# shresthasagar/quantized_spectrum_cartography

Measured on AMD Instinct MI355X. Metric: MLE grad-steps/sec + SLF NMSE, 512x512x256 R=8, higher is better.
Workload: dtype f32

## Files before the change

quantized_spectrum_cartography_amd/csrc/qsc_pass.cuh:

```cuda
#pragma once
#include <algorithm>

#include "qsc_common.cuh"

using namespace qsc;

namespace {

#if QSC_DEBUG
__device__ int g_qsc_dbg_line = 0;
inline int dbg_line_read(bool clear) {
  int line = 0;
  if (hipMemcpyFromSymbol(&line, HIP_SYMBOL(g_qsc_dbg_line), sizeof(int)) != hipSuccess) return -2;
  if (clear && line) {
    const int zero = 0;
    if (hipMemcpyToSymbol(HIP_SYMBOL(g_qsc_dbg_line), &zero, sizeof(int)) != hipSuccess) return -2;
  }
  return line;
}
#endif

constexpr int kSBlock = 256;
constexpr int kSWaves = kSBlock / 64;
#ifndef QSC_CPASS_BLOCK
#define QSC_CPASS_BLOCK 512
#endif
constexpr int kCBlock = QSC_CPASS_BLOCK;
constexpr int kCParts = kCBlock / 64;
#ifndef QSC_CPART_MIN_CHUNKS
#define QSC_CPART_MIN_CHUNKS 1.5
#endif
constexpr int kFBlock = 1024;

#ifndef QSC_SPASS_WAVES
#define QSC_SPASS_WAVES 4
#endif
#ifndef QSC_EARLY_WAVES
#define QSC_EARLY_WAVES 16
#endif
__device__ __forceinline__ void prio_level(int lvl) {
  if (lvl >= 3)
    __builtin_amdgcn_s_setprio(3);
  else if (lvl == 2)
    __builtin_amdgcn_s_setprio(2);
  else if (lvl == 1)
    __builtin_amdgcn_s_setprio(1);
  else
    __builtin_amdgcn_s_setprio(0);
}
#ifndef QSC_FUSED_WAVES
#define QSC_FUSED_WAVES 16
#endif
#ifndef QSC_CPASS_WAVES
#define QSC_CPASS_WAVES 4
#endif
struct PartRange {
  int j0, j1, js;
};
__device__ inline PartRange part_range(int W4, int p, int np) {
  return PartRange{(W4 * p) / np, (W4 * (p + 1)) / np, 1};
}
#ifndef QSC_CPASS_TILE
#define QSC_CPASS_TILE 1
#endif
#ifndef QSC_CTILE_MAXW
#define QSC_CTILE_MAXW 16
#endif
#ifndef QSC_CTILE_W16
#define QSC_CTILE_W16 8
#endif
#ifndef QSC_CTILE_SREG
#define QSC_CTILE_SREG 4
#endif
#ifndef QSC_CTILE_CT
#define QSC_CTILE_CT 1
#endif
template <int RP, int W>
struct Occ {
  static constexpr int v = (RP > 8) ? (W > 4 ? 4 : W) : W;
};
#ifndef QSC_SPASS_BPC8
#define QSC_SPASS_BPC8 3
#endif
template <int RP, int EB, int W>
struct OccS {
  static constexpr int v = (RP > 8) ? (W > 2 ? 2 : W) : (RP == 8) ? QSC_SPASS_BPC8 : W;
};

template <int RP>
struct Pitch {
  static constexpr int v = (RP == 4) ? 4 : RP + 4;
};
template <int RP, int KIND>
// ... 327 lines not shown
#pragma unroll
    for (int j = 0; j < RP / 2; ++j) acc[j] = fma2(splat2(gb), ob[j], acc[j]);
  }
}

template <int RP, typename E, int KIND, bool LOG>
__device__ __forceinline__ void half_chunk(const typename Ent<E>::V2& v, const f2v (&own)[RP / 2],
                                           const float* __restrict__ tab,
                                           const float2* __restrict__ edges, const Lik& lk,
                                           f2v (&acc)[RP / 2], f2v& nll) {
  uint32_t e[2];
  Ent<E>::unpack2(v, e);
  f2v oa[RP / 2], ob[RP / 2];
  f2v tha, thb, pq;
  pair_rows<RP, E, KIND, 0>(e[0], e[1], own, tab, oa, ob, tha, thb, lk);
  pair_math<RP, E, KIND, LOG>(e[0], e[1], own, oa, ob, tha, thb, edges, lk, acc, nll, pq);
}

constexpr int kGroup = 4;
constexpr int kSchedQ = 16;

template <typename V4>
__device__ __forceinline__ void load_group(const V4* __restrict__ src, uint32_t lo, int row, int jb,
                                           int js, int jlast, V4 (&b)[kGroup]) {
#pragma unroll
  for (int i = 0; i < kGroup; ++i) {
    const int j = min(jb + i * js, jlast);
    b[i] = ld_lane(src + (int64_t)j * row, lo);
  }
}

template <int RP, typename E, int KIND, bool LOG>
__device__ __forceinline__ void walk_groups(const typename Ent<E>::V4* __restrict__ src,
                                            uint32_t lo, int row, int jb, int j1, int js,
                                            typename Ent<E>::V4 (&b)[kGroup],
                                            const f2v (&own)[RP / 2],
                                            const float* __restrict__ tab,
                                            const float2* __restrict__ edges, const Lik& lk,
                                            f2v (&acc)[RP / 2], f2v& nll) {
  using V4 = typename Ent<E>::V4;
  const int jlast = max(j1 - 1, 0);
  const int jfirst = jb, jspan = max(j1 - jb, 1);
  auto fair = [&]() { prio_level(3 - min(3, (4 * (jb - jfirst)) / jspan)); };
  const uint32_t off = sr_addr<E, KIND>() ? lds_off(tab) : 0u;
  f2v ra[RP / 2], rb[RP / 2];
  f2v tra, trb;
  {
    uint32_t e[4];
    ent_rows4<RP, E, KIND>(b[0], off, e);
    pair_rows<RP, E, KIND, 1>(e[0], e[1], own, tab, ra, rb, tra, trb, lk);
  }
  for (;;) {
    fair();
    const int jn = jb + kGroup * js;
    const bool more = jn < j1;
    V4 nb[kGroup];
    load_group(src, lo, row, jn, js, jlast, nb);
#pragma unroll
    for (int i = 0; i < kGroup; ++i)
      if (jb + i * js < j1) {
        uint32_t e[4];
        ent_rows4<RP, E, KIND>(b[i], off, e);
        f2v xa[RP / 2], xb[RP / 2];
        f2v txa, txb, pqa, pqb;
        pair_rows<RP, E, KIND, 1>(e[2], e[3], own, tab, xa, xb, txa, txb, lk);
        pair_math<RP, E, KIND, LOG>(e[0], e[1], own, ra, rb, tra, trb, edges, lk, acc, nll, pqa);
        if (i + 1 < kGroup) {
          uint32_t f[4];
          ent_rows4<RP, E, KIND>(b[i + 1], off, f);
          pair_rows<RP, E, KIND, 1>(f[0], f[1], own, tab, ra, rb, tra, trb, lk);
        }
        pair_math<RP, E, KIND, LOG>(e[2], e[3], own, xa, xb, txa, txb, edges, lk, acc, nll, pqb);
        if constexpr (is_sr(KIND)) {
          const f2v pp = pqa * pqb;
          nll.x -= __builtin_amdgcn_logf(pp.x * pp.y);
        }
      }
    if (!more) break;
#pragma unroll
    for (int i = 0; i < kGroup; ++i) b[i] = nb[i];
    {
      uint32_t e[4];
      ent_rows4<RP, E, KIND>(b[0], off, e);
      pair_rows<RP, E, KIND, 1>(e[0], e[1], own, tab, ra, rb, tra, trb, lk);
    }
    jb = jn;
  }
}

constexpr int kGroupS = 8;

template <int RP, typename E, int KIND, bool LOG>
__device__ __forceinline__ void walk_halves(const typename Ent<E>::V2* __restrict__ src,
// ... 67 lines not shown
  do {                                                                               \
    if ((threadIdx.x & 63) == 0 && (w) < kStampWaves && (i) < kStamps)               \
      g_stamps[(w) * kStamps + (i)] = __builtin_amdgcn_s_memrealtime();              \
  } while (0)
#else
#define STAMP(w, i) \
  do {              \
  } while (0)
#define RSTAMP(w, i) \
  do {               \
  } while (0)
#endif

__device__ __forceinline__ float dpp_f(float x, int ctrl) {
  switch (ctrl) {
    case 0xB1: return __int_as_float(__builtin_amdgcn_mov_dpp(__float_as_int(x), 0xB1, 0xF, 0xF, false));
    case 0x4E: return __int_as_float(__builtin_amdgcn_mov_dpp(__float_as_int(x), 0x4E, 0xF, 0xF, false));
    case 0x141: return __int_as_float(__builtin_amdgcn_mov_dpp(__float_as_int(x), 0x141, 0xF, 0xF, false));
    default: return __int_as_float(__builtin_amdgcn_mov_dpp(__float_as_int(x), 0x140, 0xF, 0xF, false));
  }
}
__device__ __forceinline__ float wave_sum_dpp(float x) {
  x += dpp_f(x, 0xB1);
  x += dpp_f(x, 0x4E);
  x += dpp_f(x, 0x141);
  x += dpp_f(x, 0x140);
  const float a = __int_as_float(__builtin_amdgcn_readlane(__float_as_int(x), 0));
  const float b = __int_as_float(__builtin_amdgcn_readlane(__float_as_int(x), 16));
  const float c = __int_as_float(__builtin_amdgcn_readlane(__float_as_int(x), 32));
  const float d = __int_as_float(__builtin_amdgcn_readlane(__float_as_int(x), 48));
  return ((a + b) + c) + d;
}

__device__ __forceinline__ float half_sum_pick(float x, float y) {
  const auto r = __builtin_amdgcn_permlane32_swap(__float_as_uint(x), __float_as_uint(y), false,
                                                  false);
  return __uint_as_float(r[0]) + __uint_as_float(r[1]);
}
__device__ __forceinline__ float swap_lo(float x, float y) {
  const auto r = __builtin_amdgcn_permlane32_swap(__float_as_uint(x), __float_as_uint(y), false,
                                                  false);
  return __uint_as_float(r[0]);
}

__device__ __forceinline__ float cnorm_sq(const float* __restrict__ C, int n, float* sh) {
  float s2 = 0.0f;
  if (threadIdx.x < 256)
    for (int i0 = threadIdx.x; i0 < n; i0 += 8 * 256) {
      float v[8];
#pragma unroll
      for (int j = 0; j < 8; ++j) v[j] = C[min(i0 + 256 * j, n - 1)];
#pragma unroll
      for (int j = 0; j < 8; ++j)
        if (i0 + 256 * j < n) s2 = __builtin_fmaf(v[j], v[j], s2);
    }
  return block_sum(s2, sh);
}

template <int N>
__device__ __forceinline__ void ld_row(const float* __restrict__ src, float (&v)[N]) {
  if constexpr (N == 2) {
    const float2 x = *reinterpret_cast<const float2*>(src);
    v[0] = x.x;
    v[1] = x.y;
  } else {
#pragma unroll
// ... 131 lines not shown
```

quantized_spectrum_cartography_amd/csrc/qsc_pass_c.hip:

```cpp
#include "qsc_pass_host.cuh"

namespace {

template <int RP, typename E, int KIND, bool LOG>
__global__ void __launch_bounds__(kCBlock, (Occ<RP, QSC_CPASS_WAVES>::v)) cpass_kernel(
    const E* __restrict__ ent, const int* __restrict__ width, const int64_t* __restrict__ off,
    const int* __restrict__ kmap, int nks, int PT, int xcd_map, Lik lk, Edges E_, int nbins,
    int R, int K,
    const float* __restrict__ S, const float* __restrict__ C, float* __restrict__ slab,
    float* __restrict__ part_nll, float* __restrict__ cnsq) {
  using T = Ent<E>;
  using V4 = typename T::V4;
  constexpr int SP = TP<RP, KIND>::v;
  extern __shared__ __attribute__((aligned(16))) float smem[];
  float* Sl = smem;
  float2* El = reinterpret_cast<float2*>(Sl + (size_t)table_floats<RP, KIND>(PT));
  float* Pl = Sl + (size_t)table_floats<RP, KIND>(PT) + 2 * 256;
  float* Nl = Pl + (size_t)kCParts * R * 64;
  int t, ks;
  if (xcd_map) {
    const int j = blockIdx.x >> 3, x = blockIdx.x & 7;
    t = (j / nks) * 8 + x;
    ks = j - (j / nks) * nks;
  } else {
// ... 14 lines not shown
  const uint32_t lo = (uint32_t)lane * (uint32_t)sizeof(V4);
  V4 buf[kGroup];
  load_group(src, lo, 64, j0, pr.js, max(j1 - 1, 0), buf);
  const int k = kmap[wi * 64 + lane];
  float cv[RP];
#pragma unroll
  for (int r = 0; r < RP; ++r) cv[r] = C[(int64_t)min(r, R - 1) * K + min(k, K - 1)];

  {
    const float4* __restrict__ src4 = reinterpret_cast<const float4*>(S);
    constexpr int V = RP / 4;
    const int nt = gridDim.x / nks;
#pragma unroll 4
    for (int i = threadIdx.x; i < PT * V; i += kCBlock) {
      const int ql = i / V, c = i - ql * V;
      put_row4<RP, KIND>(Sl, PT, ql, 4 * c, src4[tile_pos(t, ql, nt) * V + c], lk.ob_thr);
    }
    put_pad_row<RP, KIND>(Sl, PT);
  }
  for (int i = threadIdx.x; i < nbins; i += kCBlock) El[i] = E_.e[i];
  __syncthreads();
  STAMP(wg, 1);

  const float own_scale = own_scale_of<KIND, LOG>(lk);
  f2v own[RP / 2];
#pragma unroll
  for (int j = 0; j < RP / 2; ++j)
    own[j] = f2v{(2 * j < R && k < K) ? cv[2 * j] : 0.0f,
                 (2 * j + 1 < R && k < K) ? cv[2 * j + 1] : 0.0f} * splat2(own_scale);
  f2v accp[RP / 2];
#pragma unroll
  for (int j = 0; j < RP / 2; ++j) accp[j] = splat2(0.0f);
  f2v nll = splat2(0.0f);
  walk_groups<RP, E, KIND, LOG>(src, lo, 64, j0, j1, pr.js, buf, own, Sl, El, lk, accp, nll);
  STAMP(wg, 2);
  const float nll_w = wave_sum_dpp(nll.x + nll.y) * kLn2;
#pragma unroll
  for (int j = 0; j < RP / 2; ++j) {
    if (2 * j < R) Pl[((size_t)part * R + 2 * j) * 64 + lane] = accp[j].x;
    if (2 * j + 1 < R) Pl[((size_t)part * R + 2 * j + 1) * 64 + lane] = accp[j].y;
  }
  if (lane == 0) Nl[part] = nll_w;
  __syncthreads();
  STAMP(wg, 3);

  for (int i = threadIdx.x; i < R * 64; i += kCBlock) {
    float a = Pl[i];
#pragma unroll
    for (int pp = 1; pp < kCParts; ++pp) a += Pl[(size_t)pp * R * 64 + i];
    const int r = i >> 6, l = i & 63;
    slab[((int64_t)t * R + r) * Kp + kmap[wi * 64 + l]] = a;
  }
  if (threadIdx.x == 0) {
    float a = Nl[0];
#pragma unroll
    for (int pp = 1; pp < kCParts; ++pp) a += Nl[pp];
    part_nll[wi] = a;
  }
  if (blockIdx.x == 0) {
    const float nsq = cnorm_sq(C, R * K, Nl);
    if (threadIdx.x == 0) *cnsq = nsq;
  }
  STAMP(wg, kStampLast);
  RSTAMP(wg, 29);
}

constexpr int kCTBlock = 1024;
template <int RP>
struct CTBlock {
  static constexpr int w = RP > 8 ? QSC_CTILE_W16 : kCTBlock / 64;
  static constexpr int v = 64 * w;
};

template <int RP, typename E, int KIND, bool LOG>
__global__ void __launch_bounds__(CTBlock<RP>::v) cpass_tile_kernel(
    const E* __restrict__ ent, const int* __restrict__ width, const int64_t* __restrict__ off,
    const int* __restrict__ kmap, int nks, int NP, int PT, Lik lk, Edges E_, int nbins, int R,
    int K, int ct_in,
    const float* __restrict__ S, const float* __restrict__ C, float* __restrict__ slab,
    float* __restrict__ part_nll, float* __restrict__ cnsq, float* __restrict__ snsq_out) {
  using T = Ent<E>;
  using V4 = typename T::V4;
  constexpr int SP = TP<RP, KIND>::v;
  extern __shared__ __attribute__((aligned(16))) float smem[];
  const int NW = blockDim.x >> 6;
  const int U = nks * NP;
  float* Sl = smem;
  float2* El = reinterpret_cast<float2*>(Sl + (size_t)table_floats<RP, KIND>(PT));
  float* Pl = Sl + (size_t)table_floats<RP, KIND>(PT) + 2 * 256;
  float* Nl = Pl + (NP > 1 ? (size_t)U * R * 64 : 0);
  float* Ctl = Nl + ((max(U, 16) + 3) & ~3);
  const bool ct = (RP > 8 || sizeof(E) == 2) && ct_in != 0;
  const int t = blockIdx.x;
  const int Kp = nks * 64;
  const int w = __builtin_amdgcn_readfirstlane(threadIdx.x >> 6), lane = threadIdx.x & 63;
  const float own_scale = own_scale_of<KIND, LOG>(lk);
  [[maybe_unused]] const int wg = blockIdx.x * CTBlock<RP>::w + w;
  STAMP(wg, 0);
  RSTAMP(wg, 28);

  int u = w;
  V4 buf[kGroup];
  float cv[RP];
  int wi = 0, j0 = 0, j1 = 0, js = 1, k = 0;
  const V4* src = nullptr;
  const uint32_t lo = (uint32_t)lane * (uint32_t)sizeof(V4);
  auto unit_cols = [&]() {
    if (ct) {
#pragma unroll
      for (int r = 0; r < RP; r += 4) {
        const float4 q = *reinterpret_cast<const float4*>(Ctl + (size_t)min(k, K - 1) * RP + r);
        cv[r] = q.x;
        cv[r + 1] = q.y;
        cv[r + 2] = q.z;
        cv[r + 3] = q.w;
      }
    } else {
#pragma unroll
      for (int r = 0; r < RP; ++r) cv[r] = C[(int64_t)min(r, R - 1) * K + min(k, K - 1)];
    }
  };
  auto unit_begin = [&](int uu, bool cols) {
    const int ks = uu / NP, part = uu - ks * NP;
    wi = t * nks + ks;
    const int W4 = width[wi] >> 2;
    const PartRange pr = part_range(W4, part, NP);
    j0 = pr.j0;
    j1 = pr.j1;
    js = pr.js;
    src = reinterpret_cast<const V4*>(ent + off[wi]);
    QSC_DCHECK(off[wi] + (int64_t)width[wi] * 64 <= lk.dbg_ent[1]);
    load_group(src, lo, 64, j0, js, max(j1 - 1, 0), buf);
    k = kmap[wi * 64 + lane];
    QSC_DCHECK(k >= 0 && k < Kp);
    if (cols) unit_cols();
  };
  const float4* __restrict__ src4 = reinterpret_cast<const float4*>(S);
  constexpr int V = RP / 4;
  constexpr bool kSRok = QSC_CTILE_SREG > 0 && (RP > 8 || sizeof(E) == 2);
  constexpr int kSR = kSRok ? QSC_CTILE_SREG : 1;
  const bool sreg = kSRok && PT * V <= kSR * (int)blockDim.x;
  float4 srow[kSR];
  if (sreg) {
#pragma unroll
    for (int q = 0; q < kSR; ++q) {
      const int i = (int)threadIdx.x + q * (int)blockDim.x;
      const int ql = i / V, c = i - ql * V;
      if (i < PT * V) srow[q] = src4[tile_pos(t, ql, (int)gridDim.x) * V + c];
    }
  }
  constexpr int kCT = 4;
  float ctv[kCT];
  if (ct) {
#pragma unroll
    for (int q = 0; q < kCT; ++q) {
      const int i = (int)threadIdx.x + q * (int)blockDim.x;
      if (i < R * K) ctv[q] = C[i];
    }
  }
  if (u < U) unit_begin(u, !ct);

  {
    const int nt = gridDim.x;
    if (ct) {
#pragma unroll
      for (int q = 0; q < kCT; ++q) {
// ... 5 lines not shown
      }
    }
    if (sreg) {
#pragma unroll
      for (int q = 0; q < kSR; ++q) {
        const int i = (int)threadIdx.x + q * (int)blockDim.x;
        const int ql = i / V, c = i - ql * V;
        if (i < PT * V) put_row4<RP, KIND>(Sl, PT, ql, 4 * c, srow[q], lk.ob_thr);
      }
    } else {
#pragma unroll 4
      for (int i = threadIdx.x; i < PT * V; i += blockDim.x) {
        const int ql = i / V, c = i - ql * V;
        put_row4<RP, KIND>(Sl, PT, ql, 4 * c, src4[tile_pos(t, ql, nt) * V + c], lk.ob_thr);
      }
    }
    put_pad_row<RP, KIND>(Sl, PT);
  }
  for (int i = threadIdx.x; i < nbins; i += blockDim.x) El[i] = E_.e[i];
  __syncthreads();
  STAMP(wg, 1);
  if (ct && u < U) unit_cols();

  for (; u < U; u += NW) {
    f2v own[RP / 2];
#pragma unroll
    for (int j = 0; j < RP / 2; ++j)
      own[j] = f2v{(2 * j < R && k < K) ? cv[2 * j] : 0.0f,
                   (2 * j + 1 < R && k < K) ? cv[2 * j + 1] : 0.0f} * splat2(own_scale);
    f2v accp[RP / 2];
#pragma unroll
    for (int j = 0; j < RP / 2; ++j) accp[j] = splat2(0.0f);
    f2v nll = splat2(0.0f);
    walk_groups<RP, E, KIND, LOG>(src, lo, 64, j0, j1, js, buf, own, Sl, El, lk, accp, nll);
    const float nll_w = wave_sum_dpp(nll.x + nll.y) * kLn2;
    if (NP == 1) {
#pragma unroll
      for (int j = 0; j < RP / 2; ++j) {
        if (2 * j < R) slab[((int64_t)t * R + 2 * j) * Kp + k] = accp[j].x;
        if (2 * j + 1 < R) slab[((int64_t)t * R + 2 * j + 1) * Kp + k] = accp[j].y;
      }
      if (lane == 0) part_nll[wi] = nll_w;
    } else {
#pragma unroll
      for (int j = 0; j < RP / 2; ++j) {
        if (2 * j < R) Pl[((size_t)u * R + 2 * j) * 64 + lane] = accp[j].x;
        if (2 * j + 1 < R) Pl[((size_t)u * R + 2 * j + 1) * 64 + lane] = accp[j].y;
      }
      if (lane == 0) Nl[u] = nll_w;
    }
    if (u + NW < U) unit_begin(u + NW, true);
  }
  STAMP(wg, 2);

  if (snsq_out) {
    constexpr int RH = RP / 2;
    const int nsl = PT / QSC_SLICE, nt = gridDim.x;
    const int p = lane & (QSC_SLICE - 1), h = lane >> 5;
    for (int ls = w; ls < nsl; ls += NW) {
      const float* row = Sl + (size_t)(ls * QSC_SLICE + p) * SP + h * RH;
      float nsq = 0.0f;
#pragma unroll
      for (int j = 0; j < RH; ++j) nsq = __builtin_fmaf(row[j], row[j], nsq);
      nsq = wave_sum(nsq);
      if (lane == 0) snsq_out[tile_pos(t, ls * QSC_SLICE, nt) / QSC_SLICE] = nsq;
    }
  }

  if (NP > 1) {
    __syncthreads();
    STAMP(wg, 3);
    for (int i = threadIdx.x; i < nks * R * 64; i += blockDim.x) {
      const int ks = i / (R * 64), rl = i - ks * (R * 64);
      const float* p = Pl + (size_t)ks * NP * R * 64 + rl;
      float a = p[0];
      for (int pp = 1; pp < NP; ++pp) a += p[(size_t)pp * R * 64];
      const int r = rl >> 6, l = rl & 63;
      slab[((int64_t)t * R + r) * Kp + kmap[((int64_t)t * nks + ks) * 64 + l]] = a;
    }
    for (int ks = threadIdx.x; ks < nks; ks += blockDim.x) {
      float a = Nl[ks * NP];
      for (int pp = 1; pp < NP; ++pp) a += Nl[ks * NP + pp];
      part_nll[t * nks + ks] = a;
    }
  }
  if (blockIdx.x == 0) {
    __syncthreads();
    const float nsq = cnorm_sq(C, R * K, Nl);
    if (threadIdx.x == 0) *cnsq = nsq;
  }
  STAMP(wg, kStampLast);
  RSTAMP(wg, 29);
}

int cpass_impl(const qsc_obs_desc* d, const void* c_entries, const int32_t* c_width,
               const int64_t* c_off, const int32_t* c_kmap, const qsc_model* m, int32_t R,
               const float* S, const float* C, void* ws, size_t ws_bytes, void* stream, bool nsq) {
  if (!pass_args_ok(d, m, R, ws, ws_bytes) || !S || !C || !c_width || !c_off || !c_kmap ||
      (d->c_entries > 0 && !c_entries))
    return QSC_EINVAL;
  const int RP = rp_of(R);
  const int kind = lik_kind(m);
  const bool sr = d->rowfmt == 1;
  const size_t shm = cpass_lds(d, R, sr);
  PassWs w = carve(d, R, ws);
  Edges E;
  Lik lk;
  pass_lik(d, m, &E, &lk);
  hipStream_t s = STREAM(stream);
  if (QSC_CPASS_TILE) {
    const int nks = d->nks;
    int NP = 1;
    const bool tile = tile_parts(d, R, sr, &NP);
    const int U = nks * NP;
    size_t tshm = cpass_tile_lds(d->PT, R, nks, NP, sr);
    if (tile) {
// ... 61 lines not shown
```

quantized_spectrum_cartography_amd/csrc/qsc_pass_finish.hip:

```cpp
#define QSC_PASS_NO_STAMPS
#include "qsc_pass_host.cuh"

namespace {

struct Canon {
  float nll_s, nsq_s, nll_c;
};

__device__ __forceinline__ float canon_part(const float* __restrict__ x, int n, int tid, int nb) {
  float a = 0.0f;
  if (!x) return a;
  for (int i0 = tid; i0 < n; i0 += 8 * nb) {
    float v[8];
#pragma unroll
    for (int j = 0; j < 8; ++j) v[j] = x[min(i0 + j * nb, n - 1)];
#pragma unroll
    for (int j = 0; j < 8; ++j)
      if (i0 + j * nb < n) a += v[j];
  }
  return a;
}

__device__ Canon canon_totals(const float* __restrict__ nll_s, const float* __restrict__ nsq_s,
                              const float* __restrict__ nll_c, int nslices, int nc, float* sh) {
// ... 386 lines not shown
  if (!st || R < 1 || R > QSC_MAX_R || Pp < 1 || !ws || ws_bytes < 256 * sizeof(double))
    return QSC_EINVAL;
  double* part = (double*)ws;
  const int nb = 256;
  if (S) {
    hipLaunchKernelGGL(nsq_part_kernel, dim3(nb), dim3(kSBlock), 0, STREAM(stream), S,
                       (int64_t)rp_of(R) * Pp, part);
    QSC_CHECK_LAUNCH();
  } else {
    QSC_TRY(hipMemsetAsync(part, 0, nb * sizeof(double), STREAM(stream)));
  }
  hipLaunchKernelGGL(state_init_kernel, dim3(1), dim3(64), 0, STREAM(stream), st, part, nb);
  QSC_CHECK_LAUNCH();
  return QSC_OK;
}

QSC_API int64_t qsc_pass_cnsq_offset(const qsc_obs_desc* d, int32_t R) {
  if (!desc_ok(d) || R < 1 || R > QSC_MAX_R) return -1;
  const uintptr_t base = 4096;
  return (int64_t)(reinterpret_cast<uintptr_t>(carve(d, R, reinterpret_cast<void*>(base)).cnsq) -
                   base);
}

QSC_API int qsc_obs_signed_rows_ok(const qsc_obs_desc* d, int32_t R, const qsc_model* m) {
  if (!desc_ok(d) || !m || R < 1 || R > QSC_MAX_R || m->nbounds - 1 != d->nbins) return 0;
  return (is_onebit_cf(lik_kind(m)) && sr_layout_ok(d, R)) ? 1 : 0;
}

QSC_API int qsc_scpass_supported(const qsc_obs_desc* d, int32_t R) {
  if (!desc_ok(d) || R < 1 || R > 16) return 0;
  return scpass_fits(d, R, d->rowfmt == 1) ? 1 : 0;
}

QSC_API int qsc_cfinish(const qsc_obs_desc* d, int32_t R, float* C, int32_t mode, float* dC,
                        float* mC, float* vC, const qsc_adam* adam, float lambda_c,
                        const float* normsq_c_ext, qsc_state* st, float* hist,
                        int32_t hist_cap, void* ws, size_t ws_bytes, void* stream) {
  if (!desc_ok(d) || R < 1 || R > QSC_MAX_R || !C || !st || !ws || ws_bytes < ws_bytes_for(d, R))
    return QSC_EINVAL;
  if ((mode == 0 || mode == 2) && !dC) return QSC_EINVAL;
  if (mode == 1 && (!mC || !vC || !adam)) return QSC_EINVAL;
  if (mode < 0 || mode > 2) return QSC_EINVAL;
  PassWs w = carve(d, R, ws);
  qsc_adam ad{};
  if (adam) ad = *adam;
  hipLaunchKernelGGL(cfinish_kernel, dim3((unsigned)(R * d->nks + 2)), dim3(kFBlock), 0,
                     STREAM(stream), w.slab, d->ntiles, d->nks, R, d->K, C, mode, dC, mC, vC, ad,
                     lambda_c, normsq_c_ext, w.cnsq, st, w.cnll, d->ntiles * d->nks, w.snll,
                     w.snsq, d->Pp / QSC_SLICE, hist, hist_cap, w.acache + 2);
  QSC_CHECK_LAUNCH();
  return QSC_OK;
}

QSC_API int qsc_cupdate(int32_t R, int32_t K, float* C, float* mC, float* vC, const float* g,
                        const qsc_adam* adam, float lambda_c, const float* normsq_s_ext,
                        qsc_state* st, void* stream) {
  if (R < 1 || R > QSC_MAX_R || K < 1 || !C || !mC || !vC || !g || !adam || !st)
    return QSC_EINVAL;
  hipLaunchKernelGGL(cupdate_kernel, dim3(1), dim3(kFBlock), 0, STREAM(stream), R, K, C, mC, vC,
                     g, *adam, lambda_c, normsq_s_ext, st);
  QSC_CHECK_LAUNCH();
  return QSC_OK;
}

QSC_API int qsc_state_flush(const qsc_obs_desc* d, int32_t R, qsc_state* st, float* hist,
                            int32_t hist_cap, void* ws, size_t ws_bytes, void* stream) {
// ... 97 lines not shown
```

quantized_spectrum_cartography_amd/csrc/qsc_pass_fused.hip:

```cpp
#include "qsc_pass_host.cuh"

namespace {

template <int RP>
struct FusedBlock {
  static constexpr int v = RP > 8 ? 512 : 64 * QSC_FUSED_WAVES;
  static constexpr int wpe = RP > 8 ? 2 : (QSC_FUSED_WAVES + 3) / 4;
};

#define QSC_SCF_PARAMS                                                                         \
  const E *__restrict__ s_ent, const int *__restrict__ s_width, const int64_t *__restrict__ s_off, \
      const E *__restrict__ c_ent, const int *__restrict__ c_width,                                \
      const int64_t *__restrict__ c_off, const int *__restrict__ c_kmap, int nks, int NP, int PT,  \
      Lik lk, const Edges &E_, int nbins, int R, int K, float *__restrict__ S,                    \
      const float *__restrict__ C,                                                                \
      float *__restrict__ mS, float *__restrict__ vS, qsc_adam ad, float lambda_s,                \
      qsc_state *__restrict__ st, float *__restrict__ part_nll_s, float *__restrict__ part_nsq_s, \
      float *__restrict__ slab, float *__restrict__ part_nll_c, float *__restrict__ cnsq,         \
      AdamCache *__restrict__ acache
#define QSC_SCF_KPARAMS                                                                        \
  const E *__restrict__ s_ent, const int *__restrict__ s_width, const int64_t *__restrict__ s_off, \
      const E *__restrict__ c_ent, const int *__restrict__ c_width,                                \
      const int64_t *__restrict__ c_off, const int *__restrict__ c_kmap, int nks, int NP, int PT,  \
      Lik lk, Edges E_, int nbins, int R, int K, float *__restrict__ S,                           \
      const float *__restrict__ C,                                                                \
      float *__restrict__ mS, float *__restrict__ vS, qsc_adam ad, float lambda_s,                \
      qsc_state *__restrict__ st, float *__restrict__ part_nll_s, float *__restrict__ part_nsq_s, \
      float *__restrict__ slab, float *__restrict__ part_nll_c, float *__restrict__ cnsq,         \
      AdamCache *__restrict__ acache
#define QSC_SCF_ARGS                                                                            \
  s_ent, s_width, s_off, c_ent, c_width, c_off, c_kmap, nks, NP, PT, lk, E_, nbins, R, K, S, C, mS, \
      vS, ad, lambda_s, st, part_nll_s, part_nsq_s, slab, part_nll_c, cnsq, acache


template <int RP, typename E, int KIND, bool LOG>
__device__ __forceinline__ void scfused_tile(QSC_SCF_PARAMS, const int t, const int nt,
                                             const unsigned tidx) {
  using V4 = typename Ent<E>::V4;
  constexpr int CP = TP<RP, KIND>::v;
  constexpr int RH = RP / 2;
  constexpr bool ADAM = true;
  extern __shared__ __attribute__((aligned(16))) float smem[];
  Scalars& sc = *reinterpret_cast<Scalars*>(smem);
  float* Cl = smem + 8;
  float2* El = reinterpret_cast<float2*>(Cl + (size_t)table_floats<RP, KIND>(K));
  float* Sl = reinterpret_cast<float*>(El + 256);
  float* Pl = Sl + (size_t)table_floats<RP, KIND>(PT);

  const int NW = blockDim.x >> 6;
  const int U = nks * NP;
  float* Nl = Pl + (NP > 1 ? (size_t)U * R * 64 : 0);
  const int Kp = nks * 64;
  const int w = __builtin_amdgcn_readfirstlane(tidx >> 6), lane = tidx & 63;
  const int p = lane & (QSC_SLICE - 1), h = lane >> 5;
  const float own_scale = own_scale_of<KIND, LOG>(lk);
  const int nsl = PT / QSC_SLICE;
  auto local_of = [&](int n) { return n * NW + ((n & 1) ? (NW - 1 - w) : w); };
  auto global_of = [&](int i) { return i * nt + ((i & 1) ? (nt - 1 - t) : t); };
  [[maybe_unused]] const int wg = t * (FusedBlock<RP>::v / 64) + w;
  STAMP(wg, 0);
  RSTAMP(wg, 28);
#if QSC_DIAG_STAMPS
  if (lane == 0 && wg < kStampWaves) g_stamps[wg * kStamps + 26] = __builtin_amdgcn_s_getreg(0xF804);
#endif

  const int k0 = tidx;
  const int n4 = (R * K) >> 2;
  const bool cvec = (K & 3) == 0 && ((reinterpret_cast<uintptr_t>(C) & 15) == 0);
  float4 cq = make_float4(0.0f, 0.0f, 0.0f, 0.0f);
  float c0[RP];
  if (cvec) {
    cq = reinterpret_cast<const float4*>(C)[min(k0, n4 - 1)];
  } else {
#pragma unroll
    for (int r = 0; r < RP; ++r) c0[r] = C[(int64_t)min(r, R - 1) * K + min(k0, K - 1)];
  }
  const float2 e0 = stages_edges<KIND>() ? E_.e[min(k0, nbins - 1)] : float2{};
  const int nps = nks * R * 64;
  int km_pf[2];
#pragma unroll
  for (int j = 0; j < 2; ++j) {
    const int i = min(k0 + j * (int)blockDim.x, nps - 1);
    const int ks = i / (R * 64), l = (i - ks * (R * 64)) & 63;
    km_pf[j] = c_kmap[((int64_t)t * nks + ks) * 64 + l];
  }
  float nsq_s = 0.0f;
  int step_s = 0;
  AdamCache ac0{}, ac1{};
  if (tidx == 0) {
    nsq_s = st->normsq_s;
    step_s = st->step_s;
    ac0 = acache[0];
    ac1 = acache[1];
  }
  __builtin_amdgcn_sched_barrier(0);
  STAMP(wg, 13);
  int il = local_of(0);
  SliceIn<RP, E, ADAM> cur;
  const SliceLane ln = slice_lane<RP, E>(p, h);
  const bool early = w < QSC_EARLY_WAVES;
  auto stage = [&]() {
    STAMP(wg, 14);
    if (cvec) {
      const int Ko = sr_off(K);
      auto put = [&](int i, const float4& v) {
        const int f = 4 * i, r = f / K, k = f - r * K;
        Cl[k * CP + r] = v.x;
        Cl[(k + 1) * CP + r] = v.y;
        Cl[(k + 2) * CP + r] = v.z;
        Cl[(k + 3) * CP + r] = v.w;
        if constexpr (is_sr(KIND)) {
          Cl[(Ko + k) * CP + r] = -v.x;
          Cl[(Ko + k + 1) * CP + r] = -v.y;
          Cl[(Ko + k + 2) * CP + r] = -v.z;
          Cl[(Ko + k + 3) * CP + r] = -v.w;
        }
      };
      if (k0 < n4) put(k0, cq);
// ... 102 lines not shown
    }
    float a[RH], pv[RH], m[RH], v[RH];
#pragma unroll
    for (int j = 0; j < RH; ++j) {
      a[j] = half_sum_pick(acc[j], acc[RH + j]);
      pv[j] = swap_lo(sv[j], sv[RH + j]);
      m[j] = c.mv[j];
      v[j] = c.vv[j];
    }
    float nsq = adam_row_fast<RH>(pv, m, v, a, sc.coef, sc.as, ad.project_nonneg != 0);
    const int64_t blk = (int64_t)s * QSC_SLICE * RP;
    st_row_wt<RH>(S + blk, ln.half, pv);
    st_row_wt<RH>(mS + blk, ln.half, m);
    st_row_wt<RH>(vS + blk, ln.half, v);
    st_row<RH>(Sl + (il * QSC_SLICE + p) * CP + h * RH, pv);
    if constexpr (is_sr(KIND)) {
      float nv[RH];
#pragma unroll
      for (int j = 0; j < RH; ++j) nv[j] = -pv[j];
      st_row<RH>(Sl + (sr_off(PT) + il * QSC_SLICE + p) * CP + h * RH, nv);
    }
    nsq = wave_sum_dpp(nsq);
    if (lane == 0) part_nsq_s[s] = nsq;
    const float nll_w = wave_sum_dpp(nll.x + nll.y) * kLn2;
    if (lane == 0) part_nll_s[s] = nll_w;
    STAMP(wg, 5 + min(n, 8));
    il = il1;
    ++n;
    return more;
  };
  int u = w;
  V4 buf[kGroup];
  float cv[RP];
  int wi = 0, jb = 0, je = 0, js = 1, k = 0;
  const V4* src = nullptr;
  const uint32_t lo = (uint32_t)lane * (uint32_t)sizeof(V4);
  auto unit_begin = [&](int uu) {
    const int ks = uu / NP, part = uu - ks * NP;
    wi = t * nks + ks;
    const int W4 = c_width[wi] >> 2;
    const PartRange pr = part_range(W4, part, NP);
    jb = pr.j0;
    je = pr.j1;
    js = pr.js;
    src = reinterpret_cast<const V4*>(c_ent + c_off[wi]);
    QSC_DCHECK(c_off[wi] + (int64_t)c_width[wi] * 64 <= lk.dbg_ent[1]);
    load_group(src, lo, 64, jb, js, max(pr.j1 - 1, 0), buf);
    k = c_kmap[wi * 64 + lane];
    QSC_DCHECK(k >= 0 && k < Kp);
#pragma unroll
    for (int r = 0; r < RP; ++r) cv[r] = Cl[min(k, K - 1) * CP + r];
  };
  f2v cnll = splat2(0.0f);
  auto unit_walk = [&](f2v (&accp)[RP / 2]) {
    f2v own[RP / 2];
#pragma unroll
    for (int j = 0; j < RP / 2; ++j)
      own[j] = f2v{(2 * j < R && k < K) ? cv[2 * j] : 0.0f,
                   (2 * j + 1 < R && k < K) ? cv[2 * j + 1] : 0.0f} * splat2(own_scale);
#pragma unroll
    for (int j = 0; j < RP / 2; ++j) accp[j] = splat2(0.0f);
    walk_groups<RP, E, KIND, LOG>(src, lo, 64, jb, je, js, buf, own, Sl, El, lk, accp, cnll);
  };
  auto to_pl = [&](const f2v (&accp)[RP / 2]) {
#pragma unroll
    for (int j = 0; j < RP / 2; ++j) {
      if (2 * j < R) Pl[((size_t)u * R + 2 * j) * 64 + lane] = accp[j].x;
      if (2 * j + 1 < R) Pl[((size_t)u * R + 2 * j + 1) * 64 + lane] = accp[j].y;
    }
  };

  if (il < nsl) {
    SliceIn<RP, E, ADAM> nxt;
    const bool more = one_slice(cur, nxt);
    if (more)
      for (;;) {
        if (!one_slice(nxt, cur)) break;
        if (!one_slice(cur, nxt)) break;
      }
  }

  if (t == 0 && tidx == 0) adam_cache_store(acache, ad, step_s + 2);

  STAMP(wg, 2);
  if (u < U) unit_begin(u);
  __syncthreads();
  STAMP(wg, 3);
  for (; u < U; u += NW) {
    f2v accp[RP / 2];
    unit_walk(accp);
    const float nll_w = wave_sum_dpp(cnll.x + cnll.y) * kLn2;
    cnll = splat2(0.0f);
    if (NP == 1) {
#pragma unroll
      for (int j = 0; j < RP / 2; ++j) {
        if (2 * j < R) slab[((int64_t)t * R + 2 * j) * Kp + k] = accp[j].x;
        if (2 * j + 1 < R) slab[((int64_t)t * R + 2 * j + 1) * Kp + k] = accp[j].y;
      }
      if (lane == 0) part_nll_c[wi] = nll_w;
    } else {
      to_pl(accp);
      if (lane == 0) Nl[u] = nll_w;
    }
    if (u + NW < U) unit_begin(u + NW);
  }
  STAMP(wg, 4);
  if (NP > 1) {
    __syncthreads();
    for (int i = tidx, j = 0; i < nks * R * 64; i += blockDim.x, ++j) {
      const int ks = i / (R * 64), rl = i - ks * (R * 64);
      const float* pp0 = Pl + (size_t)ks * NP * R * 64 + rl;
      float acc = pp0[0];
      for (int pp = 1; pp < NP; ++pp) acc += pp0[(size_t)pp * R * 64];
      const int r = rl >> 6, l = rl & 63;
      const int kk = j == 0 ? km_pf[0] : j == 1 ? km_pf[1] : c_kmap[((int64_t)t * nks + ks) * 64 + l];
      slab[((int64_t)t * R + r) * Kp + kk] = acc;
    }
    for (int ks = tidx; ks < nks; ks += blockDim.x) {
      float acc = Nl[ks * NP];
      for (int pp = 1; pp < NP; ++pp) acc += Nl[ks * NP + pp];
      part_nll_c[t * nks + ks] = acc;
    }
  }
  STAMP(wg, kStampLast);
  RSTAMP(wg, 29);
}

template <int RP, typename E, int KIND, bool LOG>
__global__ void __launch_bounds__(FusedBlock<RP>::v, FusedBlock<RP>::wpe)
scfused_kernel(QSC_SCF_KPARAMS) {
  scfused_tile<RP, E, KIND, LOG>(QSC_SCF_ARGS, (int)blockIdx.x, (int)gridDim.x, threadIdx.x);
}

}

#if QSC_DEBUG
int qsc::dbg_line_fused(bool clear) { return dbg_line_read(clear); }
#endif

extern "C" {

QSC_API int qsc_scpass(const qsc_obs_desc* d, const void* s_entries, const int32_t* s_width,
                       const int64_t* s_off, const void* c_entries, const int32_t* c_width,
                       const int64_t* c_off, const int32_t* c_kmap, const qsc_model* m,
                       int32_t R, float* S,
                       const float* C, float* mS, float* vS, const qsc_adam* adam,
                       float lambda_s, qsc_state* st, void* ws, size_t ws_bytes, void* stream) {
  if (!pass_args_ok(d, m, R, ws, ws_bytes) || !qsc_scpass_supported(d, R) || !S || !C || !mS ||
      !vS || !adam || !st || !s_width || !s_off || !c_width || !c_off || !c_kmap ||
      (d->s_entries > 0 && !s_entries) || (d->c_entries > 0 && !c_entries))
    return QSC_EINVAL;
  const int RP = rp_of(R);
  const int kind = lik_kind(m);
  const bool sr = d->rowfmt == 1;
// ... 31 lines not shown
```

quantized_spectrum_cartography_amd/csrc/qsc_pass_host.cuh:

```cuda
#pragma once
#include "qsc_pass.cuh"

namespace {

inline int tpitch(int R, bool sr) {
  const int RP = R <= 4 ? 4 : (R <= 8 ? 8 : 16);
  return (sr || RP > 4) ? RP + 4 : 4;
}
inline size_t trows(int rows, bool sr) { return sr ? (size_t)sr_rows(rows) : (size_t)rows; }
inline size_t tfloats(int rows, int R, bool sr) { return trows(rows, sr) * tpitch(R, sr); }

size_t cpass_tile_lds(int PT, int R, int nks, int NP, bool sr) {
  const size_t U = (size_t)nks * NP;
  return tfloats(PT, R, sr) * 4 + 2 * 256 * 4 + (NP > 1 ? U * R * 64 * 4 : 0) +
         std::max<size_t>(U, 16) * 4;
}

size_t scfused_lds(int PT, int R, int K, int nks, int NP, bool sr) {
  const size_t U = (size_t)nks * NP;
  return 32 + tfloats(K, R, sr) * 4 + 256 * 8 + tfloats(PT, R, sr) * 4 +
         (NP > 1 ? U * R * 64 * 4 : 0) + std::max<size_t>(U, 16) * 4;
}

#ifndef QSC_R16_UNITS
#define QSC_R16_UNITS 8
#endif
bool tile_parts(const qsc_obs_desc* d, int R, bool sr, int* np) {
  const int nks = d->nks;
  const int maxu = R > 8 ? QSC_R16_UNITS : QSC_CTILE_MAXW;
  int NP = nks >= maxu ? 1 : maxu / nks;
  const double chunks = (double)d->nnz / ((double)d->ntiles * d->K) / 4.0;
  const bool fused = scfused_lds(d->PT, R, d->K, nks, 1, true) <= 160 * 1024;
  while (NP > 1 && (chunks / NP < QSC_CPART_MIN_CHUNKS ||
                    cpass_tile_lds(d->PT, R, nks, NP, true) > 160 * 1024 ||
                    (fused && scfused_lds(d->PT, R, d->K, nks, NP, true) > 160 * 1024)))
    --NP;
  *np = NP;
  return QSC_CPASS_TILE && nks * NP >= 4 && cpass_tile_lds(d->PT, R, nks, NP, sr) <= 160 * 1024;
}

struct PassWs {
  float* slab;
  float* cnll;
  float* snll;
  float* snsq;
  double* init;
  int* sched;
  float* cnsq;
  AdamCache* acache;
};

inline size_t al(size_t x) { return (x + 255) & ~(size_t)255; }

PassWs carve(const qsc_obs_desc* d, int R, void* ws) {
  char* w = (char*)ws;
  PassWs p;
  const int64_t Kp = (int64_t)d->nks * 64;
  p.slab = (float*)w;
  w += al((size_t)d->ntiles * R * Kp * 4);
  p.cnll = (float*)w;
  w += al((size_t)d->ntiles * d->nks * 4);
  p.snll = (float*)w;
  w += al((size_t)(d->Pp / QSC_SLICE) * 4);
  p.snsq = (float*)w;
  w += al((size_t)(d->Pp / QSC_SLICE) * 4);
  p.init = (double*)w;
  w += al(256 * 8);
  p.sched = (int*)w;
  w += al((kSchedQ + 1) * 4);
// ... 163 lines not shown
```

Measured before the change: 61630.

## Split bin-list chunks across lanes within a wave and reduce parts via DPP

Changes the C-pass partitioning so each wave's lanes split a bin list's chunk range across NP lane groups, instead of giving each part to a separate wave unit. Partial column gradients are combined with DPP cross-lane sums in registers, which removes the LDS partial-sum buffer and the post-barrier reduction loop over R*64 entries. NP is now restricted to powers of two. The trade-off is that each wave covers fewer bins, adds DPP reduction instructions, and its memory access pattern changes.

```diff
diff --git a/quantized_spectrum_cartography_amd/csrc/qsc_pass.cuh b/quantized_spectrum_cartography_amd/csrc/qsc_pass.cuh
--- a/quantized_spectrum_cartography_amd/csrc/qsc_pass.cuh
+++ b/quantized_spectrum_cartography_amd/csrc/qsc_pass.cuh
@@ -27,6 +27,8 @@
 #endif
 constexpr int kCBlock = QSC_CPASS_BLOCK;
 constexpr int kCParts = kCBlock / 64;
+static_assert(kCParts == 1 || kCParts == 2 || kCParts == 4 || kCParts == 8,
+              "C-pass parts per bin list: 1, 2, 4 or 8");
 #ifndef QSC_CPART_MIN_CHUNKS
 #define QSC_CPART_MIN_CHUNKS 1.5
 #endif
@@ -59,6 +61,24 @@
 };
 __device__ inline PartRange part_range(int W4, int p, int np) {
   return PartRange{(W4 * p) / np, (W4 * (p + 1)) / np, 1};
+}
+struct LanePart {
+  int slot, part;
+  int n;
+  uint32_t lo;
+};
+template <typename V4>
+__device__ __forceinline__ LanePart lane_part(int W4, int sg, int lane, int sh) {
+  LanePart lp;
+  lp.part = lane & ((1 << sh) - 1);
+  lp.slot = (sg << (6 - sh)) + (lane >> sh);
+  const int j0 = (W4 * lp.part) >> sh;
+  lp.n = ((W4 * (lp.part + 1)) >> sh) - j0;
+  lp.lo = (uint32_t)(j0 * 64 + lp.slot) * (uint32_t)sizeof(V4);
+  return lp;
+}
+__device__ __forceinline__ int lane_part_max(int W4, int sh) {
+  return W4 - ((W4 * ((1 << sh) - 1)) >> sh);
 }
 #ifndef QSC_CPASS_TILE
 #define QSC_CPASS_TILE 1
@@ -452,7 +472,7 @@
 
 template <int RP, typename E, int KIND, bool LOG>
 __device__ __forceinline__ void walk_groups(const typename Ent<E>::V4* __restrict__ src,
-                                            uint32_t lo, int row, int jb, int j1, int js,
+                                            uint32_t lo, int row, int jb, int j1, int js, int nl,
                                             typename Ent<E>::V4 (&b)[kGroup],
                                             const f2v (&own)[RP / 2],
                                             const float* __restrict__ tab,
@@ -478,7 +498,7 @@
     load_group(src, lo, row, jn, js, jlast, nb);
 #pragma unroll
     for (int i = 0; i < kGroup; ++i)
-      if (jb + i * js < j1) {
+      if (jb + i * js < nl) {
         uint32_t e[4];
         ent_rows4<RP, E, KIND>(b[i], off, e);
         f2v xa[RP / 2], xb[RP / 2];
@@ -612,6 +632,47 @@
   return ((a + b) + c) + d;
 }
 
+template <int CTRL>
+__device__ __forceinline__ float dpp_c(float x) {
+  return __int_as_float(__builtin_amdgcn_mov_dpp(__float_as_int(x), CTRL, 0xF, 0xF, false));
+}
+template <int NP>
+__device__ __forceinline__ float lane_part_sum(float a) {
+  static_assert(NP == 2 || NP == 4 || NP == 8, "parts per bin in one wave: 2, 4 or 8");
+  float acc = a + dpp_c<0xF5>(a);
+  if constexpr (NP >= 4) {
+    acc += dpp_c<0xAA>(a);
+    acc += dpp_c<0xFF>(a);
+  }
+  if constexpr (NP == 8) {
+    const float m = dpp_c<0x141>(a);
+    acc += dpp_c<0xFF>(m);
+    acc += dpp_c<0xAA>(m);
+    acc += dpp_c<0x55>(m);
+    acc += m;
+  }
+  return acc;
+}
+template <int RP>
+__device__ __forceinline__ void lane_part_sum_row(const f2v (&accp)[RP / 2], int NP,
+                                                  float (&v)[RP]) {
+#pragma unroll
+  for (int j = 0; j < RP / 2; ++j) {
+    v[2 * j] = accp[j].x;
+    v[2 * j + 1] = accp[j].y;
+  }
+  if (NP == 2) {
+#pragma unroll
+    for (int r = 0; r < RP; ++r) v[r] = lane_part_sum<2>(v[r]);
+  } else if (NP == 4) {
+#pragma unroll
+    for (int r = 0; r < RP; ++r) v[r] = lane_part_sum<4>(v[r]);
+  } else if (NP == 8) {
+#pragma unroll
+    for (int r = 0; r < RP; ++r) v[r] = lane_part_sum<8>(v[r]);
+  }
+}
+
 __device__ __forceinline__ float half_sum_pick(float x, float y) {
   const auto r = __builtin_amdgcn_permlane32_swap(__float_as_uint(x), __float_as_uint(y), false,
                                                   false);
diff --git a/quantized_spectrum_cartography_amd/csrc/qsc_pass_c.hip b/quantized_spectrum_cartography_amd/csrc/qsc_pass_c.hip
--- a/quantized_spectrum_cartography_amd/csrc/qsc_pass_c.hip
+++ b/quantized_spectrum_cartography_amd/csrc/qsc_pass_c.hip
@@ -70,7 +70,7 @@
 #pragma unroll
   for (int j = 0; j < RP / 2; ++j) accp[j] = splat2(0.0f);
   f2v nll = splat2(0.0f);
-  walk_groups<RP, E, KIND, LOG>(src, lo, 64, j0, j1, pr.js, buf, own, Sl, El, lk, accp, nll);
+  walk_groups<RP, E, KIND, LOG>(src, lo, 64, j0, j1, pr.js, j1, buf, own, Sl, El, lk, accp, nll);
   STAMP(wg, 2);
   const float nll_w = wave_sum_dpp(nll.x + nll.y) * kLn2;
 #pragma unroll
@@ -125,9 +125,9 @@
   const int U = nks * NP;
   float* Sl = smem;
   float2* El = reinterpret_cast<float2*>(Sl + (size_t)table_floats<RP, KIND>(PT));
-  float* Pl = Sl + (size_t)table_floats<RP, KIND>(PT) + 2 * 256;
-  float* Nl = Pl + (NP > 1 ? (size_t)U * R * 64 : 0);
-  float* Ctl = Nl + ((max(U, 16) + 3) & ~3);
+  float* Nl = Sl + (size_t)table_floats<RP, KIND>(PT) + 2 * 256;
+  const int sh = 31 - __builtin_clz(NP);
+  float* Ctl = Nl + (((NP > 1 ? U * 64 : max(U, 16)) + 3) & ~3);
   const bool ct = (RP > 8 || sizeof(E) == 2) && ct_in != 0;
   const int t = blockIdx.x;
   const int Kp = nks * 64;
@@ -140,9 +140,9 @@
   int u = w;
   V4 buf[kGroup];
   float cv[RP];
-  int wi = 0, j0 = 0, j1 = 0, js = 1, k = 0;
+  int wi = 0, jn = 0, nl = 0, k = 0;
   const V4* src = nullptr;
-  const uint32_t lo = (uint32_t)lane * (uint32_t)sizeof(V4);
+  uint32_t lo = 0;
   auto unit_cols = [&]() {
     if (ct) {
 #pragma unroll
@@ -159,17 +159,17 @@
     }
   };
   auto unit_begin = [&](int uu, bool cols) {
-    const int ks = uu / NP, part = uu - ks * NP;
+    const int ks = uu >> sh, sg = uu - (ks << sh);
     wi = t * nks + ks;
     const int W4 = width[wi] >> 2;
-    const PartRange pr = part_range(W4, part, NP);
-    j0 = pr.j0;
-    j1 = pr.j1;
-    js = pr.js;
+    const LanePart lp = lane_part<V4>(W4, sg, lane, sh);
+    jn = lane_part_max(W4, sh);
+    nl = lp.n;
+    lo = lp.lo;
     src = reinterpret_cast<const V4*>(ent + off[wi]);
     QSC_DCHECK(off[wi] + (int64_t)width[wi] * 64 <= lk.dbg_ent[1]);
-    load_group(src, lo, 64, j0, js, max(j1 - 1, 0), buf);
-    k = kmap[wi * 64 + lane];
+    load_group(src, lo, 64, 0, 1, max(jn - 1, 0), buf);
+    k = kmap[wi * 64 + lp.slot];
     QSC_DCHECK(k >= 0 && k < Kp);
     if (cols) unit_cols();
   };
@@ -241,22 +241,22 @@
 #pragma unroll
     for (int j = 0; j < RP / 2; ++j) accp[j] = splat2(0.0f);
     f2v nll = splat2(0.0f);
-    walk_groups<RP, E, KIND, LOG>(src, lo, 64, j0, j1, js, buf, own, Sl, El, lk, accp, nll);
-    const float nll_w = wave_sum_dpp(nll.x + nll.y) * kLn2;
+    walk_groups<RP, E, KIND, LOG>(src, lo, 64, 0, jn, 1, nl, buf, own, Sl, El, lk, accp, nll);
+    const float nll_l = nll.x + nll.y;
+    const int part = lane & (NP - 1);
     if (NP == 1) {
-#pragma unroll
-      for (int j = 0; j < RP / 2; ++j) {
-        if (2 * j < R) slab[((int64_t)t * R + 2 * j) * Kp + k] = accp[j].x;
-        if (2 * j + 1 < R) slab[((int64_t)t * R + 2 * j + 1) * Kp + k] = accp[j].y;
-      }
+      const float nll_w = wave_sum_dpp(nll_l) * kLn2;
       if (lane == 0) part_nll[wi] = nll_w;
     } else {
-#pragma unroll
-      for (int j = 0; j < RP / 2; ++j) {
-        if (2 * j < R) Pl[((size_t)u * R + 2 * j) * 64 + lane] = accp[j].x;
-        if (2 * j + 1 < R) Pl[((size_t)u * R + 2 * j + 1) * 64 + lane] = accp[j].y;
-      }
-      if (lane == 0) Nl[u] = nll_w;
+      const int ks = u >> sh, slot = ((u - (ks << sh)) << (6 - sh)) + (lane >> sh);
+      Nl[((ks << sh) + part) * 64 + slot] = nll_l;
+    }
+    float dc[RP];
+    lane_part_sum_row<RP>(accp, NP, dc);
+    if (part == 0) {
+#pragma unroll
+      for (int r = 0; r < RP; ++r)
+        if (r < R) slab[((int64_t)t * R + r) * Kp + k] = dc[r];
     }
     if (u + NW < U) unit_begin(u + NW, true);
   }
@@ -279,18 +279,13 @@
   if (NP > 1) {
     __syncthreads();
     STAMP(wg, 3);
-    for (int i = threadIdx.x; i < nks * R * 64; i += blockDim.x) {
-      const int ks = i / (R * 64), rl = i - ks * (R * 64);
-      const float* p = Pl + (size_t)ks * NP * R * 64 + rl;
-      float a = p[0];
-      for (int pp = 1; pp < NP; ++pp) a += p[(size_t)pp * R * 64];
-      const int r = rl >> 6, l = rl & 63;
-      slab[((int64_t)t * R + r) * Kp + kmap[((int64_t)t * nks + ks) * 64 + l]] = a;
-    }
-    for (int ks = threadIdx.x; ks < nks; ks += blockDim.x) {
-      float a = Nl[ks * NP];
-      for (int pp = 1; pp < NP; ++pp) a += Nl[ks * NP + pp];
-      part_nll[t * nks + ks] = a;
+    for (int ks = w; ks < nks; ks += NW) {
+      float a = 0.0f;
+      for (int pp = 0; pp < NP; ++pp) {
+        const float s = wave_sum_dpp(Nl[((ks << sh) + pp) * 64 + lane]) * kLn2;
+        a = pp == 0 ? s : a + s;
+      }
+      if (lane == 0) part_nll[t * nks + ks] = a;
     }
   }
   if (blockIdx.x == 0) {
diff --git a/quantized_spectrum_cartography_amd/csrc/qsc_pass_finish.hip b/quantized_spectrum_cartography_amd/csrc/qsc_pass_finish.hip
--- a/quantized_spectrum_cartography_amd/csrc/qsc_pass_finish.hip
+++ b/quantized_spectrum_cartography_amd/csrc/qsc_pass_finish.hip
@@ -442,6 +442,11 @@
   return scpass_fits(d, R, d->rowfmt == 1) ? 1 : 0;
 }
 
+QSC_API int qsc_cpass_parts(const qsc_obs_desc* d, int32_t R) {
+  if (!desc_ok(d) || R < 1 || R > QSC_MAX_R) return 0;
+  return cpass_parts(d, R, d->rowfmt == 1);
+}
+
 QSC_API int qsc_cfinish(const qsc_obs_desc* d, int32_t R, float* C, int32_t mode, float* dC,
                         float* mC, float* vC, const qsc_adam* adam, float lambda_c,
                         const float* normsq_c_ext, qsc_state* st, float* hist,
diff --git a/quantized_spectrum_cartography_amd/csrc/qsc_pass_fused.hip b/quantized_spectrum_cartography_amd/csrc/qsc_pass_fused.hip
--- a/quantized_spectrum_cartography_amd/csrc/qsc_pass_fused.hip
+++ b/quantized_spectrum_cartography_amd/csrc/qsc_pass_fused.hip
@@ -45,11 +45,11 @@
   float* Cl = smem + 8;
   float2* El = reinterpret_cast<float2*>(Cl + (size_t)table_floats<RP, KIND>(K));
   float* Sl = reinterpret_cast<float*>(El + 256);
-  float* Pl = Sl + (size_t)table_floats<RP, KIND>(PT);
+  float* Nl = Sl + (size_t)table_floats<RP, KIND>(PT);
 
   const int NW = blockDim.x >> 6;
   const int U = nks * NP;
-  float* Nl = Pl + (NP > 1 ? (size_t)U * R * 64 : 0);
+  const int sh = 31 - __builtin_clz(NP);
   const int Kp = nks * 64;
   const int w = __builtin_amdgcn_readfirstlane(tidx >> 6), lane = tidx & 63;
   const int p = lane & (QSC_SLICE - 1), h = lane >> 5;
@@ -76,14 +76,6 @@
     for (int r = 0; r < RP; ++r) c0[r] = C[(int64_t)min(r, R - 1) * K + min(k0, K - 1)];
   }
   const float2 e0 = stages_edges<KIND>() ? E_.e[min(k0, nbins - 1)] : float2{};
-  const int nps = nks * R * 64;
-  int km_pf[2];
-#pragma unroll
-  for (int j = 0; j < 2; ++j) {
-    const int i = min(k0 + j * (int)blockDim.x, nps - 1);
-    const int ks = i / (R * 64), l = (i - ks * (R * 64)) & 63;
-    km_pf[j] = c_kmap[((int64_t)t * nks + ks) * 64 + l];
-  }
   float nsq_s = 0.0f;
   int step_s = 0;
   AdamCache ac0{}, ac1{};
@@ -252,21 +244,21 @@
   int u = w;
   V4 buf[kGroup];
   float cv[RP];
-  int wi = 0, jb = 0, je = 0, js = 1, k = 0;
+  int wi = 0, jn = 0, nl = 0, k = 0;
   const V4* src = nullptr;
-  const uint32_t lo = (uint32_t)lane * (uint32_t)sizeof(V4);
+  uint32_t lo = 0;
   auto unit_begin = [&](int uu) {
-    const int ks = uu / NP, part = uu - ks * NP;
+    const int ks = uu >> sh, sg = uu - (ks << sh);
     wi = t * nks + ks;
     const int W4 = c_width[wi] >> 2;
-    const PartRange pr = part_range(W4, part, NP);
-    jb = pr.j0;
-    je = pr.j1;
-    js = pr.js;
+    const LanePart lp = lane_part<V4>(W4, sg, lane, sh);
+    jn = lane_part_max(W4, sh);
+    nl = lp.n;
+    lo = lp.lo;
     src = reinterpret_cast<const V4*>(c_ent + c_off[wi]);
     QSC_DCHECK(c_off[wi] + (int64_t)c_width[wi] * 64 <= lk.dbg_ent[1]);
-    load_group(src, lo, 64, jb, js, max(pr.j1 - 1, 0), buf);
-    k = c_kmap[wi * 64 + lane];
+    load_group(src, lo, 64, 0, 1, max(jn - 1, 0), buf);
+    k = c_kmap[wi * 64 + lp.slot];
     QSC_DCHECK(k >= 0 && k < Kp);
 #pragma unroll
     for (int r = 0; r < RP; ++r) cv[r] = Cl[min(k, K - 1) * CP + r];
@@ -280,14 +272,7 @@
                    (2 * j + 1 < R && k < K) ? cv[2 * j + 1] : 0.0f} * splat2(own_scale);
 #pragma unroll
     for (int j = 0; j < RP / 2; ++j) accp[j] = splat2(0.0f);
-    walk_groups<RP, E, KIND, LOG>(src, lo, 64, jb, je, js, buf, own, Sl, El, lk, accp, cnll);
-  };
-  auto to_pl = [&](const f2v (&accp)[RP / 2]) {
-#pragma unroll
-    for (int j = 0; j < RP / 2; ++j) {
-      if (2 * j < R) Pl[((size_t)u * R + 2 * j) * 64 + lane] = accp[j].x;
-      if (2 * j + 1 < R) Pl[((size_t)u * R + 2 * j + 1) * 64 + lane] = accp[j].y;
-    }
+    walk_groups<RP, E, KIND, LOG>(src, lo, 64, 0, jn, 1, nl, buf, own, Sl, El, lk, accp, cnll);
   };
 
   if (il < nsl) {
@@ -309,37 +294,35 @@
   for (; u < U; u += NW) {
     f2v accp[RP / 2];
     unit_walk(accp);
-    const float nll_w = wave_sum_dpp(cnll.x + cnll.y) * kLn2;
+    const float nll_l = cnll.x + cnll.y;
     cnll = splat2(0.0f);
+    const int part = lane & (NP - 1);
     if (NP == 1) {
-#pragma unroll
-      for (int j = 0; j < RP / 2; ++j) {
-        if (2 * j < R) slab[((int64_t)t * R + 2 * j) * Kp + k] = accp[j].x;
-        if (2 * j + 1 < R) slab[((int64_t)t * R + 2 * j + 1) * Kp + k] = accp[j].y;
-      }
+      const float nll_w = wave_sum_dpp(nll_l) * kLn2;
       if (lane == 0) part_nll_c[wi] = nll_w;
     } else {
-      to_pl(accp);
-      if (lane == 0) Nl[u] = nll_w;
+      const int ks = u >> sh, slot = ((u - (ks << sh)) << (6 - sh)) + (lane >> sh);
+      Nl[((ks << sh) + part) * 64 + slot] = nll_l;
+    }
+    float dc[RP];
+    lane_part_sum_row<RP>(accp, NP, dc);
+    if (part == 0) {
+#pragma unroll
+      for (int r = 0; r < RP; ++r)
+        if (r < R) slab[((int64_t)t * R + r) * Kp + k] = dc[r];
     }
     if (u + NW < U) unit_begin(u + NW);
   }
   STAMP(wg, 4);
   if (NP > 1) {
     __syncthreads();
-    for (int i = tidx, j = 0; i < nks * R * 64; i += blockDim.x, ++j) {
-      const int ks = i / (R * 64), rl = i - ks * (R * 64);
-      const float* pp0 = Pl + (size_t)ks * NP * R * 64 + rl;
-      float acc = pp0[0];
-      for (int pp = 1; pp < NP; ++pp) acc += pp0[(size_t)pp * R * 64];
-      const int r = rl >> 6, l = rl & 63;
-      const int kk = j == 0 ? km_pf[0] : j == 1 ? km_pf[1] : c_kmap[((int64_t)t * nks + ks) * 64 + l];
-      slab[((int64_t)t * R + r) * Kp + kk] = acc;
-    }
-    for (int ks = tidx; ks < nks; ks += blockDim.x) {
-      float acc = Nl[ks * NP];
-      for (int pp = 1; pp < NP; ++pp) acc += Nl[ks * NP + pp];
-      part_nll_c[t * nks + ks] = acc;
+    for (int ks = w; ks < nks; ks += NW) {
+      float acc = 0.0f;
+      for (int pp = 0; pp < NP; ++pp) {
+        const float s = wave_sum_dpp(Nl[((ks << sh) + pp) * 64 + lane]) * kLn2;
+        acc = pp == 0 ? s : acc + s;
+      }
+      if (lane == 0) part_nll_c[t * nks + ks] = acc;
     }
   }
   STAMP(wg, kStampLast);
diff --git a/quantized_spectrum_cartography_amd/csrc/qsc_pass_host.cuh b/quantized_spectrum_cartography_amd/csrc/qsc_pass_host.cuh
--- a/quantized_spectrum_cartography_amd/csrc/qsc_pass_host.cuh
+++ b/quantized_spectrum_cartography_amd/csrc/qsc_pass_host.cuh
@@ -10,16 +10,18 @@
 inline size_t trows(int rows, bool sr) { return sr ? (size_t)sr_rows(rows) : (size_t)rows; }
 inline size_t tfloats(int rows, int R, bool sr) { return trows(rows, sr) * tpitch(R, sr); }
 
+inline size_t nll_floats(int nks, int NP) {
+  const size_t U = (size_t)nks * NP;
+  return NP > 1 ? U * 64 : std::max<size_t>(U, 16);
+}
+
 size_t cpass_tile_lds(int PT, int R, int nks, int NP, bool sr) {
-  const size_t U = (size_t)nks * NP;
-  return tfloats(PT, R, sr) * 4 + 2 * 256 * 4 + (NP > 1 ? U * R * 64 * 4 : 0) +
-         std::max<size_t>(U, 16) * 4;
+  return tfloats(PT, R, sr) * 4 + 2 * 256 * 4 + nll_floats(nks, NP) * 4;
 }
 
 size_t scfused_lds(int PT, int R, int K, int nks, int NP, bool sr) {
-  const size_t U = (size_t)nks * NP;
   return 32 + tfloats(K, R, sr) * 4 + 256 * 8 + tfloats(PT, R, sr) * 4 +
-         (NP > 1 ? U * R * 64 * 4 : 0) + std::max<size_t>(U, 16) * 4;
+         nll_floats(nks, NP) * 4;
 }
 
 #ifndef QSC_R16_UNITS
@@ -28,13 +30,14 @@
 bool tile_parts(const qsc_obs_desc* d, int R, bool sr, int* np) {
   const int nks = d->nks;
   const int maxu = R > 8 ? QSC_R16_UNITS : QSC_CTILE_MAXW;
-  int NP = nks >= maxu ? 1 : maxu / nks;
+  int NP = 1;
+  while (NP < 8 && 2 * NP * nks <= maxu) NP *= 2;
   const double chunks = (double)d->nnz / ((double)d->ntiles * d->K) / 4.0;
   const bool fused = scfused_lds(d->PT, R, d->K, nks, 1, true) <= 160 * 1024;
   while (NP > 1 && (chunks / NP < QSC_CPART_MIN_CHUNKS ||
                     cpass_tile_lds(d->PT, R, nks, NP, true) > 160 * 1024 ||
                     (fused && scfused_lds(d->PT, R, d->K, nks, NP, true) > 160 * 1024)))
-    --NP;
+    NP /= 2;
   *np = NP;
   return QSC_CPASS_TILE && nks * NP >= 4 && cpass_tile_lds(d->PT, R, nks, NP, sr) <= 160 * 1024;
 }
```

After: 60610. 0.984x the previous value.
